# nbip/IWAE

Hardware: AMD Instinct MI355X
Metric: images/sec (train step) IWAE k=50 batch 1024 @1/2/4/8 GPU; test LLH@k=5000 (higher is better)
Workload: dtype bf16; 1 GPU; 1-layer IWAE k=50 batch 1024 per GPU (BASELINE configs[1]; N=8 is configs[4]), objective iwae_elbo, train step = forward + backward + Adam(eps=1e-4); config_id=c1, global_batch=1024, n_samples=50, parallelism=dp1, rccl_ranks=0, settle_steps=100, full=False

## Files before the change

iwae_amd/csrc/kernels.h:

```cpp
#pragma once
#include <hip/hip_runtime.h>
#include <stdint.h>

namespace iwae {

#define IWAE_DENSE_G1_DEFAULT 29u
enum { EPI_TANH = 0, EPI_HEAD = 1, EPI_DX = 2, EPI_F32 = 3, EPI_BERN = 4, EPI_SIGMOID = 5 };
enum { OBJ_VAE_ELBO = 0, OBJ_IWAE_ELBO = 1, OBJ_IWAE_EQ14 = 2, OBJ_VAE_ELBO_KL = 3, OBJ_DREG = 4 };
enum { PB_LME = 0, PB_MEAN, PB_EQ14, PB_KL, PB_PX, PB_T1, PB_T2, PB_DREG, PB_COUNT };
enum { SC_VAE_ELBO = 0, SC_VAE_ELBO_KL, SC_IWAE_ELBO, SC_IWAE_EQ14, SC_INFERENCE_LOSS, SC_MEAN_LPXZ, SC_MEAN_T1, SC_MEAN_T2, SC_KL, SC_COUNT = 16 };

struct EpsSrc {
    const float* user = nullptr;
    const float* cache = nullptr;
    int ldC = 0;
    int B = 0;
    uint64_t seed = 0;
    uint64_t row_offset = 0;
    uint32_t step = 0;
    uint32_t stream = 0;
    int k_total = 0, s_off = 0, kc = 0;
};

struct LseArgs {
// ... 98 lines not shown
};
struct BlockBwdArgs {
    const uint16_t* DH; int ldDH;
    const char *imgH, *imgL2;
    int KTH, KT1, NT1;
    int R;
    const uint16_t *H2, *H1; int ldH;
    uint16_t *D2, *D1;
    int lat_on;
    LatentBwdArgs lat;
    int rows_per_wg;
};
bool block_bwd_ok(const BlockBwdArgs& a);
void launch_block_bwd(const BlockBwdArgs& a, hipStream_t st);
bool block_fwd_ok(const BlockFwdArgs& a);
bool block_fwd_shape_ok(const BlockFwdArgs& a);
void launch_block_fwd(const BlockFwdArgs& a, hipStream_t st);

struct OutBwdArgs {
    const uint16_t* G2; int ldG;
    const char* img1;
    const char* img2;
    int Xdim; int Xp32;
    const float* gx;
    const uint16_t* XB; int ldXB; int k;
    int M, KT, NG;
    uint16_t* DLP;
    const uint16_t* SP;
    float* part; int gpb;
    uint16_t* DPP;
    unsigned long long* stamps;
    int dbg;
};

struct DecBwdArgs {
    OutBwdArgs o;
    const char* imgB2;
    const uint16_t* G1;
    uint16_t* D1P;
    const char* imgB1; int MG1;
    float* DZ; int ldDZ;
    uint16_t* DZH;
    int nw;
};

struct WgradPArgs {
    const uint16_t* X; int ldX; int IT;
    const uint16_t* G; int ldG; int JT;
    int M, rows_per_split;
    float* slabW;
    float* slabB;
    const char* zero;
    const float* rowscale;
    int dbg;
    unsigned long long* stamps;
};

#define WGR_MAX_JOBS 6
struct WgradRowsJob {
    const uint16_t* X; int ldX;
    const uint16_t* G; int ldG;
    int R;
    const float* rowscale;
    int sub0, sub1, split;
    int ib, jb, wg_begin;
};
struct WgradPGroup {
    WgradPArgs a[3];
    int n;
    int gx[3], gy[3];
    int zbeg[4];
};

struct Chain2FwdArgs {
    uint16_t* Z1P;
    float* lqz1x;
    const char *e_img1, *e_img2, *e_imgh;
    const char *d_img1, *d_img2, *d_imgh;
    int M, k, B, D0, D1;
    uint16_t *EH1, *EH2;
    float* EHEAD;
    uint16_t* Z2P;
    uint16_t *DH1, *DH2;
    float* DHEAD;
    const float* head1; int ldH1;
    EpsSrc eps1, eps2;
    float *lpz1z2, *lpz2, *lqz2z1;
};
bool chain2_fwd_ok(int KT0, int KTH, int KT1, int M);
void launch_chain2_fwd(const Chain2FwdArgs& a, hipStream_t st);

struct GBlockBwdArgs {
    const char* imgH;
    const char *imgBh, *imgB2, *imgB1;
    const uint16_t *H2, *H1;
    const float* gx;
    int M, k, B, D;
    EpsSrc eps;
    const float* head1; int ldH1;
    const float* DZIN;
    uint16_t* DHP;
    uint16_t *D2P, *D1P;
    float* DZ2;
    uint16_t* DZD;
    const float* DZDEC;
    int ldDZDEC;
// ... 354 lines not shown
```

iwae_amd/csrc/kernels.hip:

```cpp
#include <hip/hip_runtime.h>
#include <hip/hip_ext.h>
#include <stdint.h>
#include <string.h>
#include <type_traits>
#include <algorithm>
#include "kernels.h"
#include "layout.h"
#include "device_helpers.h"

#ifdef IWAE_DIAG
#define WG_DBG(a, bit) (((a).dbg & (bit)) != 0)
#else
#define WG_DBG(a, bit) false
#endif
namespace iwae {

__device__ __forceinline__ void eps4(const EpsSrc& e, int b, int s, int row, int d4, int D, float n[4]) {
    if (e.cache) {
        const float4 v = *(const float4*)(e.cache + (size_t)row * e.ldC + 4 * d4);
        n[0] = v.x; n[1] = v.y; n[2] = v.z; n[3] = v.w;
    } else if (e.user) {
        const float* p = e.user + ((size_t)s * e.B + b) * D + 4 * d4;
#pragma unroll
        for (int i = 0; i < 4; ++i) n[i] = (4 * d4 + i < D) ? p[i] : 0.0f;
// ... 2905 lines not shown
            }
        }
    }
}

template <int NW, int IGC, int AI, int BJ, bool SC>
__global__ __launch_bounds__(NW * 64, (AI * BJ > 16) ? 2 : NW / 4) void wgradp_kernel(WgradPArgs a) {
    int bx = blockIdx.x, by = blockIdx.y, bz = blockIdx.z;
    const int gx = gridDim.x, gy = gridDim.y, nb = gx * gy * (int)gridDim.z;
    if ((nb & 7) == 0) {
        const int L = bx + gx * (by + gy * bz);
        const int V = (L & 7) * (nb >> 3) + (L >> 3);
        bx = V % gx; by = (V / gx) % gy; bz = V / (gx * gy);
    }
    wgradp_body<NW, IGC, AI, BJ, SC>(a, bx, by, bz);
}

__device__ __forceinline__ void wait_vmem_but_ws(int n) {
#define IWAE_WS_CASE(k) case k: asm volatile("s_waitcnt vmcnt(" #k ")" ::: "memory"); break;
    switch (n) {
        IWAE_WS_CASE(0) IWAE_WS_CASE(1) IWAE_WS_CASE(2) IWAE_WS_CASE(3) IWAE_WS_CASE(4) IWAE_WS_CASE(5) IWAE_WS_CASE(6) IWAE_WS_CASE(7)
        IWAE_WS_CASE(8) IWAE_WS_CASE(9) IWAE_WS_CASE(10) IWAE_WS_CASE(11) IWAE_WS_CASE(12) IWAE_WS_CASE(13) IWAE_WS_CASE(14) IWAE_WS_CASE(15)
        IWAE_WS_CASE(16) IWAE_WS_CASE(17) IWAE_WS_CASE(18) IWAE_WS_CASE(19) IWAE_WS_CASE(20) IWAE_WS_CASE(21) IWAE_WS_CASE(22) IWAE_WS_CASE(23)
        default: asm volatile("s_waitcnt vmcnt(24)" ::: "memory"); break;
    }
#undef IWAE_WS_CASE
}
#ifdef IWAE_DENSE_STAMPS
#define WS_STAMP(slot)                                                                 \
    {                                                                                  \
        unsigned long long t_;                                                         \
        __builtin_amdgcn_sched_barrier(0);                                             \
        asm volatile("s_memtime %0\n\ts_waitcnt lgkmcnt(0)" : "=s"(t_)::"memory");     \
        __builtin_amdgcn_sched_barrier(0);                                             \
        ws_sum[slot] += t_ - ws_prev;                                                  \
        ws_prev = t_;                                                                  \
    }
#define WS_STAMP_OUT()                                                                                                         \
    if (a.stamps && lane == 0) {                                                                                               \
        for (int i_ = 0; i_ < 8; ++i_) a.stamps[((size_t)sid * (NCW + NLW) + wave) * 8 + i_] = ws_sum[i_];                     \
    }
#else
#define WS_STAMP(slot)
#define WS_STAMP_OUT()
#endif
__device__ __forceinline__ void wgradws_block(int& bx, int& bz, const int gx, const int nz) {
    const int nb = gx * nz;
    if ((nb & 7) == 0) {
        const int L = bx + gx * bz;
        const int V = (L & 7) * (nb >> 3) + (L >> 3);
        bx = V % gx; bz = V / gx;
    }
}
template <bool SC, int BJ, int NLW>
__device__ __forceinline__ void wgradws_body(const WgradPArgs& a, const int jt0, const int bz, const int sid) {
    extern __shared__ __attribute__((aligned(1024))) char smem[];
#ifdef IWAE_DENSE_STAMPS
    unsigned long long ws_sum[8] = {0, 0, 0, 0, 0, 0, 0, 0}, ws_prev = 0;
    asm volatile("s_memtime %0\n\ts_waitcnt lgkmcnt(0)" : "=s"(ws_prev)::"memory");
#endif
    constexpr int AI = 7, IGC = 2, NCW = 8, STRIP = 4 * BJ;
    constexpr int XT_BYTES = WG_SR * 512, GROW = STRIP * 32, GT_BYTES = WG_SR * GROW, BUF = XT_BYTES + GT_BYTES;
    constexpr int XP = XT_BYTES / 1024, GP = GT_BYTES / 1024, XPL = XP / NLW, GPL = GP / NLW, PPL = XPL + GPL;
    constexpr int SPR = GROW / 16, RPP = 1024 / GROW;
    static_assert(XP % NLW == 0 && GP % NLW == 0 && GPL >= 1 && GPL <= 4, "loader split");
    typedef __attribute__((ext_vector_type(4))) short v4s;
    auto gswz = [](int r) { return SPR >= 16 ? ((r & 3) << 2) : (((r >> 1) & 1) << 2); };
    const int tid = threadIdx.x, lane = tid & 63, wave = __builtin_amdgcn_readfirstlane(tid >> 6);
    const int rbeg = bz * a.rows_per_split;
    const int rend = min(a.M, rbeg + a.rows_per_split);
    const int nstage = (rend - rbeg + WG_SR - 1) / WG_SR;
    const int gcol0 = jt0 * 16;

    if (SC && wave >= NCW) {
        typedef __attribute__((ext_vector_type(4))) uint32_t u32x4;
        __builtin_amdgcn_s_setprio(3);
        const int lw = wave - NCW;
        const char* zsrc = a.zero + (lane & 31) * 16;
        const int xstride = WG_SR * a.ldX * 2, gstride = WG_DBG(a, 32) ? 0 : WG_SR * a.ldG * 2;
        const char* xbase[XPL]; int xlim[XPL];
#pragma unroll
        for (int i = 0; i < XPL; ++i) {
            const int pc = lw * XPL + i, rl = 2 * pc + (lane >> 5);
            const int col = ((lane & 31) ^ ((rl & 3) << 2)) * 8;
            xbase[i] = (const char*)a.X + ((size_t)(rbeg + rl) * a.ldX + col) * 2;
            xlim[i] = col < a.ldX ? rend - rbeg - rl : -(1 << 30);
        }
        const char* gbase[GPL]; int glim[GPL];
#pragma unroll
        for (int i = 0; i < GPL; ++i) {
            const int pc = lw * GPL + i, rl = RPP * pc + lane / SPR;
            const int col = gcol0 + ((lane % SPR) ^ gswz(rl)) * 8;
            const bool ok = col < a.ldG;
            gbase[i] = (const char*)a.G + ((size_t)(rbeg + rl) * a.ldG + (ok ? col : 0)) * 2;
            glim[i] = ok ? rend - rbeg - rl : -(1 << 30);
        }
        constexpr int NR = RPP * GPL;
        static_assert(NR == 8 || NR == 4, "row weights of a loader and stage are one s_load_dwordx8 / x4");
        typedef __attribute__((ext_vector_type(NR))) float wvec_t;
        auto load_w = [&](int st, wvec_t& w) {
            const uint64_t ad = (uint64_t)(a.rowscale + (rbeg + st * WG_SR + NR * lw));
            const uint64_t au = ((uint64_t)(uint32_t)__builtin_amdgcn_readfirstlane((int)(uint32_t)(ad >> 32)) << 32) |
                                (uint64_t)(uint32_t)__builtin_amdgcn_readfirstlane((int)(uint32_t)ad);
            if constexpr (NR == 8) asm volatile("s_load_dwordx8 %0, %1, 0x0" : "=s"(w) : "s"(au) : "memory");
            else asm volatile("s_load_dwordx4 %0, %1, 0x0" : "=s"(w) : "s"(au) : "memory");
        };
        auto wsel = [&](const wvec_t& w, int i) {
            float f = w[RPP * i];
#pragma unroll
            for (int r = 1; r < RPP; ++r) f = (lane / SPR == r) ? w[RPP * i + r] : f;
            return f;
        };
        constexpr int PER = GPL + XPL;
        u32x4 gq0[GPL], gq1[GPL], gq2[GPL], gq3[GPL];
        auto issue_g = [&](int st, int i, u32x4& dst) {
// ... 22 lines not shown
            for (int i = 0; i < XPL; ++i) issue_x(st, i);
        };
        if (0 < nstage) issue_all(0, gq0);
        if (1 < nstage) issue_all(1, gq1);
        if (2 < nstage) issue_all(2, gq2);
        wait_vmem_but_ws(per_stage(1) + per_stage(2));
        asm volatile("s_waitcnt lgkmcnt(0)" : "+s"(wcur) : : "memory");
        if (0 < nstage) {
#pragma unroll
            for (int i = 0; i < GPL; ++i) { asm volatile("" : "+v"(gq0[i])); put_piece(0, i, gq0[i], wcur); }
        }
        __syncthreads();
        WS_STAMP(0)
        auto iter = [&](int c, u32x4 (&gn)[GPL], u32x4 (&gc)[GPL]) {
            const bool next = c + 1 < nstage;
            if (next) load_w(c + 1, wcur);
            if (c + 3 < nstage) issue_all(c + 3, gn);
            WS_STAMP(1)
            if (next) {
                wait_vmem_but_ws(per_stage(c + 2) + per_stage(c + 3));
                asm volatile("s_waitcnt lgkmcnt(0)" : "+s"(wcur) : : "memory");
            }
            WS_STAMP(2)
            if (next) {
#pragma unroll
                for (int i = 0; i < GPL; ++i) { asm volatile("" : "+v"(gc[i])); put_piece(c + 1, i, gc[i], wcur); }
            }
            WS_STAMP(3)
            __syncthreads();
            WS_STAMP(4)
        };
        for (int c = 0; c < nstage; c += 4) {
            iter(c, gq3, gq1);
            if (c + 1 < nstage) iter(c + 1, gq0, gq2);
            if (c + 2 < nstage) iter(c + 2, gq1, gq3);
            if (c + 3 < nstage) iter(c + 3, gq2, gq0);
        }
        asm volatile("s_waitcnt vmcnt(0)" ::: "memory");
        WS_STAMP_OUT()
        return;
    }
    if (wave >= NCW) {
        const int lw = wave - NCW;
        const char* zsrc = a.zero + (lane & 31) * 16;
        const char* pbase[PPL];
        int plim[PPL];
        const int xstride = WG_SR * a.ldX * 2, gstride = WG_SR * a.ldG * 2;
#pragma unroll
        for (int i = 0; i < PPL; ++i) {
            const bool isx = i < XPL;
            int rl, col, ld;
            if (isx) {
                const int pc = lw * XPL + i;
                rl = 2 * pc + (lane >> 5);
                col = ((lane & 31) ^ ((rl & 3) << 2)) * 8;
                ld = a.ldX;
            } else {
                const int pc = lw * GPL + (i - XPL);
                rl = RPP * pc + lane / SPR;
                col = gcol0 + ((lane % SPR) ^ gswz(rl)) * 8;
                ld = a.ldG;
            }
            pbase[i] = (const char*)(isx ? a.X : a.G) + ((size_t)(rbeg + rl) * ld + col) * 2;
            plim[i] = col < ld ? rend - rbeg - rl : -(1 << 30);
        }
        auto issue = [&](int st) {
#pragma unroll
            for (int i = 0; i < PPL; ++i) {
                const bool isx = i < XPL;
                const int pc = isx ? lw * XPL + i : XP + lw * GPL + (i - XPL);
                const char* src = (st * WG_SR < plim[i]) ? pbase[i] + (size_t)st * (size_t)(isx ? xstride : gstride) : zsrc;
                glds16(src, (uint32_t)__builtin_amdgcn_readfirstlane((int)(lds_addr_of(smem + (st % WG_NST) * BUF) + (uint32_t)pc * 1024u)));
            }
        };
        if (0 < nstage) issue(0);
        if (1 < nstage) issue(1);
        if (2 < nstage) issue(2);
        wait_vmem_but_ws((1 < nstage ? PPL : 0) + (2 < nstage ? PPL : 0));
        __syncthreads();
        for (int c = 0; c < nstage; ++c) {
            const bool refill = c + 3 < nstage && !WG_DBG(a, 1);
            if (refill) issue(c + 3);
            if (c + 1 < nstage) wait_vmem_but_ws((c + 2 < nstage ? PPL : 0) + (refill ? PPL : 0));
            __syncthreads();
        }
        asm volatile("s_waitcnt vmcnt(0)" ::: "memory");
        return;
    }

    const int q = lane >> 4, l16 = lane & 15, qp = l16 >> 2, p = l16 & 3;
    const int ig = wave % IGC, jg = wave / IGC;
    f32x4 acc[AI][BJ], accb[BJ];
#pragma unroll
    for (int u = 0; u < BJ; ++u) {
        accb[u] = (f32x4){0.0f, 0.0f, 0.0f, 0.0f};
#pragma unroll
        for (int t = 0; t < AI; ++t) acc[t][u] = (f32x4){0.0f, 0.0f, 0.0f, 0.0f};
    }
    const int xrow_off = (4 * q + qp) * 512, grow_off = (4 * q + qp) * GROW;
    const uint4 ones = make_uint4(0x3F803F80u, 0x3F803F80u, 0x3F803F80u, 0x3F803F80u);
    const bool do_bias = ig == 0 && !WG_DBG(a, 4);
    __syncthreads();
    WS_STAMP(0)
    for (int c = 0; c < nstage; ++c) {
        const int buf = c % WG_NST;
        const char* xb = smem + buf * BUF + xrow_off + p * 16;
        const char* gbase = smem + buf * BUF + XT_BYTES + grow_off;
        uint4 g[BJ];
#pragma unroll
        for (int u = 0; u < BJ; ++u) {
            const int jl = jg * BJ + u;
            const char* gb = gbase + ((((4 * (jl >> 1)) ^ gswz(qp)) + p) * 16) + 8 * (jl & 1);
            const v4s g0 = __builtin_amdgcn_ds_read_tr16_b64_v4i16((__attribute__((address_space(3))) v4s*)gb);
            const v4s g1 = __builtin_amdgcn_ds_read_tr16_b64_v4i16((__attribute__((address_space(3))) v4s*)(gb + 16 * GROW));
            const uint2 glo = __builtin_bit_cast(uint2, g0), ghi = __builtin_bit_cast(uint2, g1);
            g[u] = make_uint4(glo.x, glo.y, ghi.x, ghi.y);
        }
        WS_STAMP(1)
        if (!WG_DBG(a, 2)) {
            lds_pipeline<AI, 3>(
                [&](int t) {
                    const int i = ig * AI + t;
                    const char* p0 = xb + ((((4 * (i >> 1)) ^ (qp << 2))) * 16) + 8 * (i & 1);
                    const v4s r0 = __builtin_amdgcn_ds_read_tr16_b64_v4i16((__attribute__((address_space(3))) v4s*)p0);
                    const v4s r1 = __builtin_amdgcn_ds_read_tr16_b64_v4i16((__attribute__((address_space(3))) v4s*)(p0 + 16 * 512));
                    const uint2 lo = __builtin_bit_cast(uint2, r0), hi = __builtin_bit_cast(uint2, r1);
                    return make_uint4(lo.x, lo.y, hi.x, hi.y);
                },
                [&](int t, const uint4& av) {
#pragma unroll
                    for (int u = 0; u < BJ; ++u) acc[t][u] = mfma16(av, g[u], acc[t][u]);
                });
        }
        if (do_bias) {
#pragma unroll
            for (int u = 0; u < BJ; ++u) accb[u] = mfma16(ones, g[u], accb[u]);
        }
        WS_STAMP(2)
        __syncthreads();
        WS_STAMP(3)
    }
    if (WG_DBG(a, 16)) return;
    float* slab = a.slabW + (size_t)bz * a.IT * 16 * a.JT * 16;
#pragma unroll
    for (int u = 0; u < BJ; ++u) {
        const int jt = jt0 + jg * BJ + u;
        if (jt < a.JT) {
#pragma unroll
            for (int t = 0; t < AI; ++t) {
                const int it = ig * AI + t;
                if (it < a.IT) {
#pragma unroll
                    for (int ii = 0; ii < 4; ++ii)
                        slab[(size_t)(it * 16 + 4 * q + ii) * (a.JT * 16) + jt * 16 + l16] = acc[t][u][ii];
                }
            }
            if (ig == 0 && q == 0) a.slabB[(size_t)bz * a.JT * 16 + jt * 16 + l16] = accb[u][0];
        }
    }
    WS_STAMP(4)
    WS_STAMP_OUT()
}

template <bool SC, int BJ, int NLW>
__global__ __launch_bounds__((8 + NLW) * 64, NLW == 8 ? 4 : 3) void wgradws_kernel(WgradPArgs a) {
    int bx = blockIdx.x, bz = blockIdx.z;
    wgradws_block(bx, bz, gridDim.x, gridDim.z);
    const int sid = bz * (int)gridDim.x + bx;
    if constexpr (BJ == 4) {
        if (bx == (int)gridDim.x - 1 && a.JT - bx * 16 <= 4 && (SC || gridDim.x > 1)) { wgradws_body<SC, 1, NLW>(a, bx * 16, bz, sid); return; }
    }
    wgradws_body<SC, BJ, NLW>(a, bx * 4 * BJ, bz, sid);
}
__global__ __launch_bounds__(768, 3) void wgradws_group_kernel(WgradPGroup g) {
    int l = 0;
    while (l + 1 < g.n && (int)blockIdx.z >= g.zbeg[l + 1]) ++l;
    if ((int)blockIdx.x >= g.gx[l]) return;
    int bx = blockIdx.x, bz = blockIdx.z - g.zbeg[l];
    wgradws_block(bx, bz, g.gx[l], g.zbeg[l + 1] - g.zbeg[l]);
    wgradws_body<false, 4, 4>(g.a[l], bx * 16, bz, 0);
}

__global__ __launch_bounds__(512, 2) void wgradp_group_kernel(WgradPGroup g) {
    int l = 0;
    while (l + 1 < g.n && (int)blockIdx.z >= g.zbeg[l + 1]) ++l;
    if ((int)blockIdx.x >= g.gx[l] || (int)blockIdx.y >= g.gy[l]) return;
    wgradp_body<8, 4, 4, 4, false>(g.a[l], blockIdx.x, blockIdx.y, blockIdx.z - g.zbeg[l]);
}
__global__ __launch_bounds__(512, 2) void wgradp_group_sc_kernel(WgradPGroup g) {
    int l = 0;
    while (l + 1 < g.n && (int)blockIdx.z >= g.zbeg[l + 1]) ++l;
    if ((int)blockIdx.x >= g.gx[l] || (int)blockIdx.y >= g.gy[l]) return;
    if (l == 0) wgradp_body<8, 4, 4, 4, true>(g.a[0], blockIdx.x, blockIdx.y, blockIdx.z);
    else wgradp_body<8, 4, 4, 4, false>(g.a[l], blockIdx.x, blockIdx.y, blockIdx.z - g.zbeg[l]);
}

__global__ __launch_bounds__(256) void prep_rows_kernel(const float* x, const float* cond, int B, int X, int C, int Xp, int Bp, uint16_t* XP) {
    const int lane = threadIdx.x & 63;
    const int b = blockIdx.x * 64 + lane;
    const int nchunk = Xp / 8;
    if (b >= Bp) return;
    for (int c = blockIdx.y * 4 + (threadIdx.x >> 6); c < nchunk; c += gridDim.y * 4) {
        const int t = c >> 2, qq = c & 3;
        float v[8];
#pragma unroll
        for (int h = 0; h < 2; ++h) {
            const int f0 = 32 * t + 16 * h + 4 * qq;
#pragma unroll
            for (int i = 0; i < 4; ++i) {
                const int f = f0 + i;
                float t = 0.0f;
                if (b < B && f < X) t = x[(size_t)b * X + f];
                else if (b < B && f < X + C) t = cond[(size_t)b * C + (f - X)];
                v[4 * h + i] = t;
            }
        }
        if (b < B) *(uint4*)(XP + (size_t)b * Xp + 8 * c) = make_uint4(pack2(v[0], v[1]), pack2(v[2], v[3]), pack2(v[4], v[5]), pack2(v[6], v[7]));
    }
}

__global__ __launch_bounds__(256) void gather_binarize_kernel(const uint8_t* data, const int32_t* order, int start, int N, int B, int X, int Xp,
                                                              int Bp, uint64_t seed, uint32_t epoch, uint16_t* XP, float* xf,
                                                              const uint8_t* labels, int C, float* cond_out) {
    const int lane = threadIdx.x & 63;
    const int b = blockIdx.x * 64 + lane;
    const int nchunk = Xp / 8;
    if (b >= Bp) return;
    const int img = (b < B) ? order[start + b] : 0;
    const int lab = (labels && b < B) ? (int)labels[img] : -1;
    if (cond_out && blockIdx.y == 0 && threadIdx.x < 64 && b < B)
        for (int j = 0; j < C; ++j) cond_out[(size_t)b * C + j] = (j == lab) ? 1.0f : 0.0f;
    for (int c = blockIdx.y * 4 + (threadIdx.x >> 6); c < nchunk; c += gridDim.y * 4) {
        const int t = c >> 2, qq = c & 3;
// ... 858 lines not shown
        const int nparts = a.part ? (a.NG + a.gpb - 1) / a.gpb : 1;
        dim3 grid((a.M + 127) / 128, nparts);
        hipEvent_t stop = g_stop_event;
        if (a.part) g_stop_event = nullptr;
        switch (a.KT) {
            case 7: LAUNCH_EV(out_bwd_s_kernel<7>, grid, dim3(256), lds, st, a); break;
            case 4: LAUNCH_EV(out_bwd_s_kernel<4>, grid, dim3(256), lds, st, a); break;
            case 2: LAUNCH_EV(out_bwd_s_kernel<2>, grid, dim3(256), lds, st, a); break;
            default: return;
        }
        if (a.part) {
            g_stop_event = stop;
            LAUNCH_EV(out_bwd_finish_kernel, grid1((size_t)a.M * (a.ldG / 8), 256), dim3(256), 0, st, a, nparts);
        }
        return;
    }
    constexpr int PAIRS = 2;
    const size_t ldsp = 2 * ((size_t)a.KT * 4096 + 1024) + (size_t)PAIRS * 4096;
    dim3 gridp((a.M + PAIRS * 32 - 1) / (PAIRS * 32));
#ifdef IWAE_DIAG
    if (a.stamps) {
        LAUNCH_EV((out_bwd_pair_kernel<7, PAIRS, true>), gridp, dim3(PAIRS * 128), 2 * ((size_t)7 * 4096 + 1024) + (size_t)PAIRS * 4096, st, a);
        return;
    }
#endif
    switch (a.KT) {
        case 7: LAUNCH_EV((out_bwd_pair_kernel<7, PAIRS, false>), gridp, dim3(PAIRS * 128), ldsp, st, a); break;
        case 4: LAUNCH_EV((out_bwd_pair_kernel<4, PAIRS, false>), gridp, dim3(PAIRS * 128), ldsp, st, a); break;
        case 2: LAUNCH_EV((out_bwd_pair_kernel<2, PAIRS, false>), gridp, dim3(PAIRS * 128), ldsp, st, a); break;
        default: {
            const size_t lds = 2 * ((size_t)a.KT * 8192 + 1024);
            LAUNCH_EV((out_bwd_kernel<0, false>), dim3((a.M + 127) / 128), dim3(256), lds, st, a);
        }
    }
}
void launch_wgradws_group(const WgradPGroup& g, hipStream_t st) {
    int mx = 0;
    for (int l = 0; l < g.n; ++l) mx = std::max(mx, g.gx[l]);
    LAUNCH_EV(wgradws_group_kernel, dim3(mx, 1, g.zbeg[g.n]), dim3(768), WG_NST * (WG_SR * 512 + WG_SR * 512), st, g);
}
void launch_wgradp_group(const WgradPGroup& g, hipStream_t st) {
    int mx = 0, my = 0;
    for (int l = 0; l < g.n; ++l) { mx = std::max(mx, g.gx[l]); my = std::max(my, g.gy[l]); }
    if (g.a[0].rowscale) hipLaunchKernelGGL(wgradp_group_sc_kernel, dim3(mx, my, g.zbeg[g.n]), dim3(512), WG_NST * (WG_SR * 512 + WG_SR * 256 + 1024), st, g);
    else hipLaunchKernelGGL(wgradp_group_kernel, dim3(mx, my, g.zbeg[g.n]), dim3(512), WG_NST * (WG_SR * 512 + WG_SR * 256), st, g);
}
int wgradp_strip(int shape) { return (shape == 8 || shape == 9) ? 8 : 16; }
void launch_wgradp(const WgradPArgs& a, int nsplit, int shape, hipStream_t st) {
    dim3 grid((a.JT + wgradp_strip(shape) - 1) / wgradp_strip(shape), (a.IT + 15) / 16, nsplit);
    const size_t sc = a.rowscale ? 1024 : 0;
    if (shape == 7) {
        const size_t lds = WG_NST * (WG_SR * 512 + WG_SR * 512);
        if (a.rowscale) LAUNCH_EV((wgradws_kernel<true, 4, 4>), grid, dim3(768), lds, st, a);
        else LAUNCH_EV((wgradws_kernel<false, 4, 4>), grid, dim3(768), lds, st, a);
    } else if (shape == 9) {
        const size_t lds = WG_NST * (WG_SR * 512 + WG_SR * 256);
        if (a.rowscale) LAUNCH_EV((wgradws_kernel<true, 2, 8>), grid, dim3(1024), lds, st, a);
        else LAUNCH_EV((wgradws_kernel<false, 2, 8>), grid, dim3(1024), lds, st, a);
    } else if (shape == 16) {
        const size_t lds = WG_NST * (WG_SR * 512 + WG_SR * 512 + sc);
        if (a.rowscale) LAUNCH_EV((wgradp_kernel<16, 2, 8, 2, true>), grid, dim3(1024), lds, st, a);
        else LAUNCH_EV((wgradp_kernel<16, 4, 4, 4, false>), grid, dim3(1024), lds, st, a);
    } else {
        const size_t lds = WG_NST * (WG_SR * 512 + WG_SR * 256 + sc);
        if (a.rowscale) LAUNCH_EV((wgradp_kernel<8, 4, 4, 4, true>), grid, dim3(512), lds, st, a);
        else LAUNCH_EV((wgradp_kernel<8, 4, 4, 4, false>), grid, dim3(512), lds, st, a);
    }
}
void launch_prep_rows(const float* x, const float* cond, int B, int X, int C, int Xp, int Bp, uint16_t* XP, hipStream_t st) {
    const int nchunk = Xp / 8;
    hipLaunchKernelGGL(prep_rows_kernel, dim3(Bp / 64, std::min(32, (nchunk + 3) / 4)), dim3(256), 0, st, x, cond, B, X, cond ? C : 0, Xp, Bp, XP);
}
void launch_gather_binarize(const uint8_t* data, const int32_t* order, int start, int N, int B, int X, int Xp, int Bp, uint64_t seed,
                            uint32_t epoch, uint16_t* XP, float* xf, hipStream_t st, const uint8_t* labels, int C, float* cond_out) {
    const int nchunk = Xp / 8;
    hipLaunchKernelGGL(gather_binarize_kernel, dim3(Bp / 64, std::min(32, (nchunk + 3) / 4)), dim3(256), 0, st, data, order, start, N, B, X, Xp,
                       Bp, seed, epoch, XP, xf, labels, labels ? C : 0, cond_out);
}
void launch_eps_gen_multi(const EpsSrc& e, int M, int D, int ld, float* out, int nsteps, size_t step_stride, hipStream_t st) {
    const int nd4 = (D + 3) / 4;
    hipLaunchKernelGGL(eps_gen_multi_kernel, grid1((size_t)nsteps * M * nd4, 256), dim3(256), 0, st, e, M, nd4, ld, out, nsteps, step_stride);
}
void launch_eps_gen(const EpsSrc& e, int M, int D, int ld, float* out, hipStream_t st, int max_blocks) {
    const int nd4 = (D + 3) / 4;
    dim3 grid = grid1((size_t)M * nd4, 256);
    if (max_blocks > 0 && (int)grid.x > max_blocks) grid.x = max_blocks;
    hipLaunchKernelGGL(eps_gen_kernel, grid, dim3(256), 0, st, e, M, nd4, ld, out);
}
void launch_sample(const SampleArgs& a, hipStream_t st) { hipLaunchKernelGGL(sample_kernel, dim3((a.M + 63) / 64), dim3(256), 0, st, a); }
void launch_gauss_lp(const GaussLpArgs& a, hipStream_t st) { hipLaunchKernelGGL(gauss_lp_kernel, dim3((a.M + 63) / 64), dim3(256), 0, st, a); }
void launch_lse(const LseArgs& a, hipStream_t st) {
    if (a.k >= 2048) LAUNCH_EV(lse_block_kernel<16>, dim3(a.B), dim3(1024), 0, st, a);
    else if (a.k > 256) LAUNCH_EV(lse_block_kernel<4>, dim3(a.B), dim3(256), 0, st, a);
    else LAUNCH_EV(lse_kernel, grid1((size_t)a.B * 64, 256), dim3(256), 0, st, a);
}
void launch_latent_bwd(const LatentBwdArgs& a, hipStream_t st) {
    if (a.dzh && !a.dz2 && a.eps.cache && !a.prior_head) hipLaunchKernelGGL(latent_bwd_kernel<1>, dim3(a.Bp), dim3(256), 0, st, a);
    else if (!a.dzh && a.dz && a.dz2 && a.dz3 && a.eps.cache && !a.prior_head) hipLaunchKernelGGL(latent_bwd_kernel<2>, dim3(a.Bp), dim3(256), 0, st, a);
    else hipLaunchKernelGGL(latent_bwd_kernel<0>, dim3(a.Bp), dim3(256), 0, st, a);
}
void launch_gauss_bwd(const GaussBwdArgs& a, hipStream_t st) {
    hipLaunchKernelGGL(gauss_bwd_kernel, grid1((size_t)a.Mp * (a.Dp / 4), 256), dim3(256), 0, st, a);
}
void launch_reduce_grads(const LayerDesc* layers, int nlayers, int first_block, int nblocks, float* grad, float* param, float* mom, float* vel,
                         float alpha, float beta1, float beta2, float eps, int fuse_adam, const float* per_b, int B, float beta, float* scalars, hipStream_t st,
                         int first_block2, int nblocks2) {
// ... 50 lines not shown
```

iwae_amd/csrc/model.h:

```cpp
#pragma once
#include <hip/hip_runtime.h>
#include <stddef.h>
#include <stdint.h>
#include <string>
#include <type_traits>
#include <vector>
#include <rccl/rccl.h>
#include "../../include/iwae_amd.h"
#include "kernels.h"

#pragma GCC visibility push(hidden)

int fail(int code, const std::string& msg);
#define HIPCHK(expr)                                                                                   \
    do {                                                                                               \
        hipError_t e_ = (expr);                                                                        \
        if (e_ != hipSuccess)                                                                          \
            return fail(e_ == hipErrorOutOfMemory ? IWAE_ERR_NOMEM : IWAE_ERR_HIP,                     \
                        std::string(#expr) + ": " + hipGetErrorString(e_));                            \
    } while (0)
#define CHK(expr) do { int rc_ = (expr); if (rc_ != IWAE_OK) return rc_; } while (0)

struct DevBuf { void* p = nullptr; size_t cap = 0; };
struct KerasLayer { std::string name; int Kin, Nout; size_t offW, offb; };
// ... 23 lines not shown

enum TimedKernel { T_OUT_BWD = 0, T_DEC_FWD, T_WGRAD_OUT, T_DX_HID, T_DX_LAT, T_WGRAD_HID, T_WGRAD_LAT, T_LATENT_BWD, T_ENC_FWD, T_REDUCE, T_DEC_BWD, T_AR_ENC, T_AR_DEC, T_AIS_CHAIN, T_LOCAL_Q, T_IMPUTE, T_COUNT };

struct FwdCall {
    uint32_t batch_offset = 0;
    int cond_row0 = 0;
    int k_total = 0, s_off = 0;
    bool log_w_only = false;
    bool no_ksplit = false;
};

struct StepOptions {
    bool allow_s_mode = true;
    bool allow_zin = true;
    bool allow_zin_eval = false;
    bool allow_eps_multi = true;
    int eps_blocks = 512;
    bool allow_block_fused = true;
    bool allow_out_in_block = true;
    bool allow_dec_fused = true;
    bool allow_bern_pipe = true;
    bool bern_qw = true;
    bool bern_qw_force = false;
    bool allow_lse_fused = true;
    bool allow_lse_dup = true;
    bool allow_lse_in_bwd = true;
    bool allow_early_wout = true;
    bool allow_g2w = false;
    bool allow_chain2 = true;
    bool allow_chain2_bwd = true;
    unsigned dense_g1_mask = IWAE_DENSE_G1_DEFAULT;
    bool allow_dec_bwd = true;
    bool small_dec_bwd = true; int small_rows = 8191;
    int dec_rows_max = 1024;
    int dec_bwd_nw = 8;
    bool allow_dz_half = true;
    bool allow_wg3 = true;
    bool allow_dec_rows = true;
    bool allow_wgrad_rows = true;
    bool allow_lat_rows4 = false;
    bool allow_lat_in_block = true;
    bool use_side2 = true;
    bool allow_wg_group = false;
    int wout_split = 0, wout_wg1 = 56, wout_wg2 = 128;
    bool defer_split = false;
    bool allow_defer = true;
    bool allow_defer2 = true;
    bool allow_defer2_split = true;
    int wg_target16 = 0;
    int wg_target16_1 = 64;
    int wg_target8 = 128;
    int wg_target8_few = 32;
    int wg_shape9 = 0;
    bool allow_wg7 = true;
    bool dp_concurrent = false;
    iwae::GemmF32Opts gemm_f32;
    bool allow_f32_multi_reduce = true;
    bool allow_f32_side = true, f32_wout_first = true;
    int f32_dw_last = 0;
    int f32_dw_min_rows = 32;
    int f32_dw_tiles = 1024;
    bool f32_dec_fused_train = false;
    bool allow_f32_dec_fused = true;
    bool allow_f32_bern_fused = true;
    int eval_rows = 0;
    int grid_chunk = 0;
    int ais_t_chunk = 0;
    int local_t_chunk = 0;
    int impute_rows = 0;
};

enum ZFrom { Z_SAMPLE = 0, Z_DENSE_ZIN, Z_DEC_PROLOGUE, Z_BLOCK, Z_CHAIN2 };
enum DecFwd { DEC_DENSE = 0, DEC_BLOCK2, DEC_BLOCK_OUT, DEC_PIPE };
enum LseAt { LSE_FWD = 0, LSE_DECODER, LSE_BWD_ROWS };
enum DxPath { DX_THREE = 0, DX_DEC_BWD, DX_ROWS };
enum OnStream { ON_MAIN = 0, ON_SIDE, ON_SIDE2 };
struct StepPlan {
    bool zin_eval = false;
    bool keep_eps = false;
    bool eps_multi = false;
    bool enc_takes_f32 = false;
    ZFrom z_from = Z_SAMPLE;
    bool chain = false;
    bool chain2_bwd = false;
    DecFwd dec_fwd = DEC_DENSE;
    iwae::DenseArgs bern;
    iwae::BlockFwdArgs dec_blk;
    int px_parts = 1;
    bool s_mode = false;
    bool early_wout = false;
    bool lse_fused = false;
    bool lse_dup = false;
    bool g2w = false;
    LseAt lse_at = LSE_FWD;
    bool want_dreg = false;
    OnStream draw_on = ON_SIDE;
    bool dec_rows = false;
    DxPath dx = DX_THREE;
    iwae::DecBwdRowsArgs rows;
    bool out_parts = false;
    bool dz_half = false;
    bool lat_fuse = false;
    bool rows_enc = false;
    bool group3 = false;
    bool wout_two_part = false;
    bool hid_group = false;
// ... 213 lines not shown
```

iwae_amd/csrc/model.hip:

```cpp
#include <math.h>
#include <stdio.h>
#include <string.h>
#include <stddef.h>
#include <stdlib.h>
#include <algorithm>
#include <random>
#include <memory>
#include <dlfcn.h>
#include "model.h"
#include "layout.h"

using namespace iwae;

static_assert(sizeof(iwae_config) == 64 && offsetof(iwae_config, struct_size) == 0 && offsetof(iwae_config, seed) == 32 && offsetof(iwae_config, cond_dim) == 48 &&
              offsetof(iwae_config, cond_prior) == 52 && offsetof(iwae_config, precision) == 56, "iwae_config layout is part of the ABI (iwae_amd/_capi.py)");
static_assert(sizeof(iwae_scalars) == 64 && sizeof(iwae_tensors) == 12 * sizeof(void*), "ABI struct layout");
static_assert(sizeof(iwae_ais_options) == 72 && offsetof(iwae_ais_options, betas) == 16 && offsetof(iwae_ais_options, step_size) == 24 && offsetof(iwae_ais_options, z0) == 40 &&
              offsetof(iwae_ais_options, unif) == 64 && sizeof(iwae_ais_outputs) == 10 * sizeof(void*), "iwae_ais_options / iwae_ais_outputs layout is part of the ABI (iwae_amd/_capi.py)");
static_assert(sizeof(iwae_local_options) == 64 && offsetof(iwae_local_options, objective) == 16 && offsetof(iwae_local_options, lr) == 20 && offsetof(iwae_local_options, epsilon) == 32 &&
              offsetof(iwae_local_options, mu0) == 40 && offsetof(iwae_local_options, eps) == 56 && sizeof(iwae_local_outputs) == 9 * sizeof(void*), "iwae_local_options / iwae_local_outputs layout is part of the ABI (iwae_amd/_capi.py)");
static_assert(sizeof(iwae_impute_options) == 24 && offsetof(iwae_impute_options, k) == 4 && offsetof(iwae_impute_options, mask) == 8 && offsetof(iwae_impute_options, eps) == 16 &&
              sizeof(iwae_impute_outputs) == 6 * sizeof(void*), "iwae_impute_options / iwae_impute_outputs layout is part of the ABI (iwae_amd/_capi.py)");

static thread_local std::string g_err;
// ... 224 lines not shown
    e.cache = m->epsc_ptr[layer];
    e.ldC = eps_ld(m, layer);
    if (m->user_eps) e.user = ptr<float>(m->epsbuf) + (layer == 0 ? 0 : (size_t)m->k * m->B * m->D[0]);
    e.B = m->B;
    e.seed = m->cfg.seed;
    e.row_offset = (uint64_t)m->call.batch_offset * (uint64_t)m->k;
    e.step = m->noise_step;
    e.stream = (uint32_t)layer;
    if (m->call.k_total > 0) {
        e.k_total = m->call.k_total; e.s_off = m->call.s_off; e.kc = m->k;
        e.row_offset = (uint64_t)m->call.batch_offset * (uint64_t)m->call.k_total;
    }
    return e;
}
namespace {

int attach_dense_stamps(iwae_model* m, int epi, DenseArgs& a) {
    if (m->dstamp_epi != epi || m->dstamp_kt != a.KT || (a.M < 4096 && a.KT <= 8)) return IWAE_OK;
    m->dstamp_waves = std::max(((a.M + 127) / 128) * ((a.MG + a.mg_per_block - 1) / a.mg_per_block) * 4, epi == EPI_BERN ? ((a.M + 127) / 128) * 16 : 0);
    CHK(ensure(m->dstamps, (size_t)m->dstamp_waves * 64, m->stream));
    a.stamps = ptr<unsigned long long>(m->dstamps);
    return IWAE_OK;
}

bool block_fwd_shape(const iwae_model* m, const Linear* blk, int R, BlockFwdArgs& a) {
    memset(&a, 0, sizeof(a));
    a.ldX = blk[0].Kp32; a.img0 = blk[0].imgF; a.img1 = blk[1].imgF; a.img2 = blk[2].imgF;
    a.KT0 = blk[0].KT; a.KT1 = blk[1].KT; a.NT1 = blk[0].Np32 / 16; a.NT2 = blk[2].Np32 / 16; a.R = R;
    a.ldH = blk[0].Np32; a.ldYF = blk[2].Np32; a.split = (blk[2].nsub == 2) ? blk[2].joff[1] : (1 << 30);
    return m->opt.allow_block_fused && blk[1].Np32 == blk[0].Np32 && blk[2].KT == blk[1].KT && blk[1].Kp32 == blk[0].Np32 && block_fwd_ok(a);
}

void wgradp_shape(const iwae_model* m, const Linear& L, int rows, int& nsplit, int& nw, int& cps) {
    const int chunks = (rows + 63) / 64;
    nw = (L.JT > 8 && chunks >= 128) ? 16 : 8;
    if (nw == 16 && L.IT <= 14 && m->opt.allow_wg7) nw = (m->opt.wg_shape9 & (L.JT > 16 ? 1 : 2)) ? 9 : 7;
    const int blocks = ((L.JT + wgradp_strip(nw) - 1) / wgradp_strip(nw)) * ((L.IT + 15) / 16);
    const int target16 = m->opt.wg_target16 > 0 ? m->opt.wg_target16 : (m->cfg.n_layers == 2 ? 64 : 96);
    const int target = (nw != 8) ? (blocks == 1 ? m->opt.wg_target16_1 : target16) : (chunks < 128 ? m->opt.wg_target8_few : m->opt.wg_target8);
    nsplit = std::max(1, std::min(chunks, target / std::max(1, blocks)));
    cps = (chunks + nsplit - 1) / nsplit;
    nsplit = (chunks + cps - 1) / cps;
}
int wgradp_plan(iwae_model* m, Linear& L, const uint16_t* XP, const uint16_t* GP, int rows, WgradPArgs& a, int& nsplit, int& nw) {
    int cps;
    wgradp_shape(m, L, rows, nsplit, nw, cps);
    const size_t needW = (size_t)nsplit * L.IT * 16 * L.JT * 16 * 4, needB = (size_t)nsplit * L.JT * 16 * 4;
    void* oldW = L.slabW.p; void* oldB = L.slabB.p;
    CHK(ensure(L.slabW, needW, m->stream));
    CHK(ensure(L.slabB, needB, m->stream));
    if (oldW != L.slabW.p || oldB != L.slabB.p || nsplit != L.nsplit) { L.nsplit = nsplit; m->descs_dirty = true; }
    a.X = XP; a.ldX = L.Kp32; a.IT = L.IT; a.G = GP; a.ldG = L.Np32; a.JT = L.JT; a.M = rows; a.rows_per_split = cps * 64;
    a.slabW = ptr<float>(L.slabW); a.slabB = ptr<float>(L.slabB); a.zero = m->d_zero; a.rowscale = nullptr;
    a.dbg = m->wg_debug;
    a.stamps = nullptr;
    return IWAE_OK;
}

int wgradp(iwae_model* m, Linear& L, const uint16_t* XP, const uint16_t* GP, int rows, hipStream_t st = nullptr,
           const float* rowscale = nullptr) {
    WgradPArgs a;
    int nsplit = 1, nw = 8;
    CHK(wgradp_plan(m, L, XP, GP, rows, a, nsplit, nw));
    a.rowscale = rowscale;
    if (rowscale && (m->fake_s & 2)) a.dbg |= 32;
#ifdef IWAE_DENSE_STAMPS
    if (m->dstamp_epi == 10 && rowscale && nw == 7) {
        m->dstamp_waves = ((L.JT + 15) / 16) * nsplit * 12;
        CHK(ensure(m->dstamps, (size_t)m->dstamp_waves * 64, m->stream));
        a.stamps = ptr<unsigned long long>(m->dstamps);
    }
#endif
    launch_wgradp(a, nsplit, nw, st ? st : m->stream);
    HIPCHK(hipGetLastError());
    return IWAE_OK;
}

int wgradp_two_plan(iwae_model* m, Linear& L, const uint16_t* XP, const uint16_t* GP, int rows, const float* rowscale, WgradPArgs& a1, int& n1, WgradPArgs& a2, int& n2) {
    const int blocks = (L.JT + 15) / 16;
    const int chunks = (rows + 63) / 64;
    const int c1 = std::min(chunks - 1, std::max(1, (int)((long)chunks * m->opt.wout_split / 100)));
    const int c2 = chunks - c1;
    auto split = [&](int ch, int target, int& n, int& cps) { n = std::max(1, std::min(ch, target / std::max(1, blocks))); cps = (ch + n - 1) / n; n = (ch + cps - 1) / cps; };
    int cps1, cps2;
    split(c1, m->opt.wout_wg1, n1, cps1);
    split(c2, m->opt.wout_wg2, n2, cps2);
    const int ns = n1 + n2;
    const size_t stride = (size_t)L.IT * 16 * L.JT * 16;
    void* oldW = L.slabW.p; void* oldB = L.slabB.p;
    CHK(ensure(L.slabW, (size_t)ns * stride * 4, m->stream));
    CHK(ensure(L.slabB, (size_t)ns * L.JT * 16 * 4, m->stream));
    if (oldW != L.slabW.p || oldB != L.slabB.p || ns != L.nsplit) { L.nsplit = ns; m->descs_dirty = true; }
    const int R1 = c1 * 64;
    memset(&a1, 0, sizeof(a1));
    a1.X = XP; a1.ldX = L.Kp32; a1.IT = L.IT; a1.G = GP; a1.ldG = L.Np32; a1.JT = L.JT; a1.M = R1; a1.rows_per_split = cps1 * 64;
    a1.slabW = ptr<float>(L.slabW); a1.slabB = ptr<float>(L.slabB); a1.zero = m->d_zero; a1.rowscale = rowscale;
    a2 = a1;
    a2.X = XP + (size_t)R1 * L.Kp32; a2.G = GP + (size_t)R1 * L.Np32; a2.M = rows - R1; a2.rows_per_split = cps2 * 64;
    a2.slabW = a1.slabW + (size_t)n1 * stride; a2.slabB = a1.slabB + (size_t)n1 * L.JT * 16; a2.rowscale = rowscale + R1;
    return IWAE_OK;
}

int dense_dx(iwae_model* m, Linear& L, const uint16_t* GP, int rows, const uint16_t* ACT, uint16_t* YP, float* YF) {
    DenseArgs a;
    memset(&a, 0, sizeof(a));
    a.X = GP; a.ldX = L.Np32; a.img = L.imgB;
// ... 1361 lines not shown
    HIPCHK(hipSetDevice(m->cfg.device));
    CHK(join_side(m));
    HIPCHK(hipStreamSynchronize(m->stream));
    if (m->side) HIPCHK(hipStreamSynchronize(m->side));
    if (m->side2) HIPCHK(hipStreamSynchronize(m->side2));
    m->have_forward = false;
    const bool on = value != 0;
    const int iv = (int)value;
    const std::string n(name);
    if (n == "out_recompute") m->opt.allow_s_mode = !on;
    else if (n == "no_defer") m->opt.allow_defer = !on;
    else if (n == "wout_split") m->opt.wout_split = std::max(0, std::min(95, iv));
    else if (n == "wout_wg1") m->opt.wout_wg1 = std::max(1, iv);
    else if (n == "wout_wg2") m->opt.wout_wg2 = std::max(1, iv);
    else if (n == "defer_split") m->opt.defer_split = on;
    else if (n == "no_eps_multi") m->opt.allow_eps_multi = !on;
    else if (n == "no_zin") m->opt.allow_zin = !on;
    else if (n == "zin_eval") m->opt.allow_zin_eval = on;
    else if (n == "no_chain2_bwd") m->opt.allow_chain2_bwd = !on;
    else if (n == "no_chain2") m->opt.allow_chain2 = !on;
    else if (n == "no_dec_bwd") m->opt.allow_dec_bwd = !on;
    else if (n == "no_defer2_split") m->opt.allow_defer2_split = !on;
    else if (n == "no_defer2") m->opt.allow_defer2 = !on;
    else if (n == "f32_dw_tiles") m->opt.f32_dw_tiles = std::max(1, iv);
    else if (n == "f32_dw_min_rows") m->opt.f32_dw_min_rows = std::max(16, iv);
    else if (n == "f32_gemm_dbg") m->opt.gemm_f32.dbg = iv;
    else if (n == "f32_gemm_small_min") m->opt.gemm_f32.v2_small_min = std::max(1, iv);
    else if (n == "f32_ksplit_min_tiles") m->opt.gemm_f32.ksplit_min_tiles = std::max(1, iv);
    else if (n == "f32_no_ksplit") m->opt.gemm_f32.ksplit = !on;
    else if (n == "f32_gemm_small_v1") m->opt.gemm_f32.v2_small = !on;
    else if (n == "f32_gemm_w4") m->opt.gemm_f32.w8 = !on;
    else if (n == "f32_gemm_v1") m->opt.gemm_f32.v2 = !on;
    else if (n == "no_f32_side") m->opt.allow_f32_side = !on;
    else if (n == "f32_dw_last") m->opt.f32_dw_last = iv;
    else if (n == "f32_wout_last") m->opt.f32_wout_first = !on;
    else if (n == "no_f32_multi_reduce") m->opt.allow_f32_multi_reduce = !on;
    else if (n == "f32_dec_fused_train") m->opt.f32_dec_fused_train = on;
    else if (n == "no_f32_dec_fused") m->opt.allow_f32_dec_fused = !on;
    else if (n == "no_f32_bern_fused") m->opt.allow_f32_bern_fused = !on;
    else if (n == "no_dec_rows") m->opt.allow_dec_rows = !on;
    else if (n == "no_wgrad_rows") m->opt.allow_wgrad_rows = !on;
    else if (n == "no_wg3") m->opt.allow_wg3 = !on;
    else if (n == "g2w") m->opt.allow_g2w = on;
    else if (n == "lat_rows4") m->opt.allow_lat_rows4 = on;
    else if (n == "no_lat_in_block") m->opt.allow_lat_in_block = !on;
    else if (n == "no_lse_in_bwd") m->opt.allow_lse_in_bwd = !on;
    else if (n == "no_lse_fused") m->opt.allow_lse_fused = !on;
    else if (n == "no_lse_dup") m->opt.allow_lse_dup = !on;
    else if (n == "dz_f32") m->opt.allow_dz_half = !on;
    else if (n == "no_small_dec_bwd") m->opt.small_dec_bwd = !on;
    else if (n == "small_rows") m->opt.small_rows = iv;
    else if (n == "dec_rows") m->opt.dec_rows_max = iv;
    else if (n == "no_wg7") m->opt.allow_wg7 = !on;
    else if (n == "wg9") m->opt.wg_shape9 = iv;
    else if (n == "grid_chunk") m->opt.grid_chunk = iv > 0 ? std::max(16, iv) : 0;
    else if (n == "ais_t_chunk") m->opt.ais_t_chunk = iv > 0 ? iv : 0;
    else if (n == "local_t_chunk") m->opt.local_t_chunk = iv > 0 ? iv : 0;
    else if (n == "impute_rows") m->opt.impute_rows = iv > 0 ? iv : 0;
    else if (n == "eval_rows") m->opt.eval_rows = iv > 0 ? std::max(64, iv) : 0;
    else if (n == "no_bern_pipe") m->opt.allow_bern_pipe = !on;
    else if (n == "no_block_fused") m->opt.allow_block_fused = !on;
    else if (n == "no_out_in_block") m->opt.allow_out_in_block = !on;
    else if (n == "no_dec_fused") m->opt.allow_dec_fused = !on;
    else if (n == "no_bern_qw") m->opt.bern_qw = !on;
    else if (n == "bern_qw_force") m->opt.bern_qw_force = on;
    else if (n == "dense_g1") m->opt.dense_g1_mask = (unsigned)iv;
    else if (n == "wg8") m->opt.wg_target8 = std::max(1, iv);
    else if (n == "wg8_few") m->opt.wg_target8_few = std::max(1, iv);
    else if (n == "wg16") m->opt.wg_target16 = std::max(1, iv);
    else if (n == "wg16_1") m->opt.wg_target16_1 = std::max(1, iv);
    else if (n == "eps_blocks") m->opt.eps_blocks = std::max(0, iv);
    else if (n == "dec_bwd_nw") m->opt.dec_bwd_nw = iv == 8 ? 8 : 4;
    else if (n == "no_side2") m->opt.use_side2 = !on;
    else if (n == "wg_group") m->opt.allow_wg_group = on;
    else if (n == "no_early_wout") m->opt.allow_early_wout = !on;
    else if (n == "dp_concurrent") m->opt.dp_concurrent = on;
#ifdef IWAE_DIAG
    else if (n == "stamps") { m->want_stamps = on; if (on) { m->opt.allow_s_mode = false; m->opt.allow_bern_pipe = false; m->opt.allow_block_fused = false; m->opt.allow_dec_fused = false; } }
    else if (n == "dense_stamps_epi") m->dstamp_epi = iv;
    else if (n == "dense_stamps_kt") m->dstamp_kt = iv;
    else if (n == "wg_debug") m->wg_debug = iv;
    else if (n == "abl_skip") m->abl_skip = iv;
    else if (n == "fake_s") m->fake_s = iv;
#endif
    else return fail(IWAE_ERR_ARG, "set_option: unknown option '" + n + "'");
    return IWAE_OK;
}

int iwae_set_eval_precision(iwae_handle m, int32_t precision) {
    if (!m) return fail(IWAE_ERR_ARG, "null handle");
    if (precision != IWAE_PREC_BF16 && precision != IWAE_PREC_FP32) return fail(IWAE_ERR_ARG, "precision must be IWAE_PREC_BF16 or IWAE_PREC_FP32");
    m->eval_precision = precision;
    return IWAE_OK;
}

int iwae_set_adam(iwae_handle m, float beta1, float beta2, float epsilon) {
    if (!m) return fail(IWAE_ERR_ARG, "null handle");
    if (!(beta1 >= 0.f && beta1 < 1.f) || !(beta2 >= 0.f && beta2 < 1.f) || !(epsilon > 0.f)) return fail(IWAE_ERR_ARG, "set_adam: need 0 <= beta < 1, epsilon > 0");
    m->adam_b1 = beta1; m->adam_b2 = beta2; m->adam_eps = epsilon;
    return IWAE_OK;
}

int iwae_train_step(iwae_handle m, const float* x, int32_t B, int32_t k, float beta, float lr, int32_t objective, const float* eps,
                    iwae_scalars* scalars, const iwae_tensors* want) {
    if (!m) return fail(IWAE_ERR_ARG, "null handle");
    HIPCHK(hipSetDevice(m->cfg.device));
// ... 487 lines not shown
```

Baseline: 5.193 million images/s.

## Add narrow-X tile variant to weight-gradient kernel for small input widths

New measurement: 5.265 million images/s (median of 6 runs). 1.01x the previous value.

```diff
diff --git a/iwae_amd/csrc/kernels.h b/iwae_amd/csrc/kernels.h
--- a/iwae_amd/csrc/kernels.h
+++ b/iwae_amd/csrc/kernels.h
@@ -174,6 +174,7 @@
     float* slabB;
     const char* zero;
     const float* rowscale;
+    int narrow_x;
     int dbg;
     unsigned long long* stamps;
 };
diff --git a/iwae_amd/csrc/kernels.hip b/iwae_amd/csrc/kernels.hip
--- a/iwae_amd/csrc/kernels.hip
+++ b/iwae_amd/csrc/kernels.hip
@@ -2981,15 +2981,18 @@
         bx = V % gx; bz = V / gx;
     }
 }
-template <bool SC, int BJ, int NLW>
+template <bool SC, int BJ, int NLW, bool NX = false>
 __device__ __forceinline__ void wgradws_body(const WgradPArgs& a, const int jt0, const int bz, const int sid) {
     extern __shared__ __attribute__((aligned(1024))) char smem[];
 #ifdef IWAE_DENSE_STAMPS
     unsigned long long ws_sum[8] = {0, 0, 0, 0, 0, 0, 0, 0}, ws_prev = 0;
     asm volatile("s_memtime %0\n\ts_waitcnt lgkmcnt(0)" : "=s"(ws_prev)::"memory");
 #endif
-    constexpr int AI = 7, IGC = 2, NCW = 8, STRIP = 4 * BJ;
-    constexpr int XT_BYTES = WG_SR * 512, GROW = STRIP * 32, GT_BYTES = WG_SR * GROW, BUF = XT_BYTES + GT_BYTES;
+    constexpr int AI = NX ? 8 : 7, IGC = NX ? 1 : 2, NCW = 8, STRIP = 4 * BJ;
+    constexpr int BJW = STRIP / (NCW / IGC);
+    constexpr int XPITCH = NX ? 256 : 512, XSL = XPITCH / 16, XRPP = 1024 / XPITCH;
+    static_assert(!NX || (!SC && BJ == 4), "the narrow X tile exists for the unweighted 8 + 4-wave shape");
+    constexpr int XT_BYTES = WG_SR * XPITCH, GROW = STRIP * 32, GT_BYTES = WG_SR * GROW, BUF = XT_BYTES + GT_BYTES;
     constexpr int XP = XT_BYTES / 1024, GP = GT_BYTES / 1024, XPL = XP / NLW, GPL = GP / NLW, PPL = XPL + GPL;
     constexpr int SPR = GROW / 16, RPP = 1024 / GROW;
     static_assert(XP % NLW == 0 && GP % NLW == 0 && GPL >= 1 && GPL <= 4, "loader split");
@@ -3118,8 +3121,8 @@
             int rl, col, ld;
             if (isx) {
                 const int pc = lw * XPL + i;
-                rl = 2 * pc + (lane >> 5);
-                col = ((lane & 31) ^ ((rl & 3) << 2)) * 8;
+                rl = XRPP * pc + lane / XSL;
+                col = ((lane % XSL) ^ ((rl & 3) << 2)) * 8;
                 ld = a.ldX;
             } else {
                 const int pc = lw * GPL + (i - XPL);
@@ -3156,14 +3159,14 @@
 
     const int q = lane >> 4, l16 = lane & 15, qp = l16 >> 2, p = l16 & 3;
     const int ig = wave % IGC, jg = wave / IGC;
-    f32x4 acc[AI][BJ], accb[BJ];
-#pragma unroll
-    for (int u = 0; u < BJ; ++u) {
+    f32x4 acc[AI][BJW], accb[BJW];
+#pragma unroll
+    for (int u = 0; u < BJW; ++u) {
         accb[u] = (f32x4){0.0f, 0.0f, 0.0f, 0.0f};
 #pragma unroll
         for (int t = 0; t < AI; ++t) acc[t][u] = (f32x4){0.0f, 0.0f, 0.0f, 0.0f};
     }
-    const int xrow_off = (4 * q + qp) * 512, grow_off = (4 * q + qp) * GROW;
+    const int xrow_off = (4 * q + qp) * XPITCH, grow_off = (4 * q + qp) * GROW;
     const uint4 ones = make_uint4(0x3F803F80u, 0x3F803F80u, 0x3F803F80u, 0x3F803F80u);
     const bool do_bias = ig == 0 && !WG_DBG(a, 4);
     __syncthreads();
@@ -3172,10 +3175,10 @@
         const int buf = c % WG_NST;
         const char* xb = smem + buf * BUF + xrow_off + p * 16;
         const char* gbase = smem + buf * BUF + XT_BYTES + grow_off;
-        uint4 g[BJ];
-#pragma unroll
-        for (int u = 0; u < BJ; ++u) {
-            const int jl = jg * BJ + u;
+        uint4 g[BJW];
+#pragma unroll
+        for (int u = 0; u < BJW; ++u) {
+            const int jl = jg * BJW + u;
             const char* gb = gbase + ((((4 * (jl >> 1)) ^ gswz(qp)) + p) * 16) + 8 * (jl & 1);
             const v4s g0 = __builtin_amdgcn_ds_read_tr16_b64_v4i16((__attribute__((address_space(3))) v4s*)gb);
             const v4s g1 = __builtin_amdgcn_ds_read_tr16_b64_v4i16((__attribute__((address_space(3))) v4s*)(gb + 16 * GROW));
@@ -3189,18 +3192,18 @@
                     const int i = ig * AI + t;
                     const char* p0 = xb + ((((4 * (i >> 1)) ^ (qp << 2))) * 16) + 8 * (i & 1);
                     const v4s r0 = __builtin_amdgcn_ds_read_tr16_b64_v4i16((__attribute__((address_space(3))) v4s*)p0);
-                    const v4s r1 = __builtin_amdgcn_ds_read_tr16_b64_v4i16((__attribute__((address_space(3))) v4s*)(p0 + 16 * 512));
+                    const v4s r1 = __builtin_amdgcn_ds_read_tr16_b64_v4i16((__attribute__((address_space(3))) v4s*)(p0 + 16 * XPITCH));
                     const uint2 lo = __builtin_bit_cast(uint2, r0), hi = __builtin_bit_cast(uint2, r1);
                     return make_uint4(lo.x, lo.y, hi.x, hi.y);
                 },
                 [&](int t, const uint4& av) {
 #pragma unroll
-                    for (int u = 0; u < BJ; ++u) acc[t][u] = mfma16(av, g[u], acc[t][u]);
+                    for (int u = 0; u < BJW; ++u) acc[t][u] = mfma16(av, g[u], acc[t][u]);
                 });
         }
         if (do_bias) {
 #pragma unroll
-            for (int u = 0; u < BJ; ++u) accb[u] = mfma16(ones, g[u], accb[u]);
+            for (int u = 0; u < BJW; ++u) accb[u] = mfma16(ones, g[u], accb[u]);
         }
         WS_STAMP(2)
         __syncthreads();
@@ -3209,8 +3212,8 @@
     if (WG_DBG(a, 16)) return;
     float* slab = a.slabW + (size_t)bz * a.IT * 16 * a.JT * 16;
 #pragma unroll
-    for (int u = 0; u < BJ; ++u) {
-        const int jt = jt0 + jg * BJ + u;
+    for (int u = 0; u < BJW; ++u) {
+        const int jt = jt0 + jg * BJW + u;
         if (jt < a.JT) {
 #pragma unroll
             for (int t = 0; t < AI; ++t) {
@@ -3228,7 +3231,7 @@
     WS_STAMP_OUT()
 }
 
-template <bool SC, int BJ, int NLW>
+template <bool SC, int BJ, int NLW, bool NX = false>
 __global__ __launch_bounds__((8 + NLW) * 64, NLW == 8 ? 4 : 3) void wgradws_kernel(WgradPArgs a) {
     int bx = blockIdx.x, bz = blockIdx.z;
     wgradws_block(bx, bz, gridDim.x, gridDim.z);
@@ -3236,7 +3239,7 @@
     if constexpr (BJ == 4) {
         if (bx == (int)gridDim.x - 1 && a.JT - bx * 16 <= 4 && (SC || gridDim.x > 1)) { wgradws_body<SC, 1, NLW>(a, bx * 16, bz, sid); return; }
     }
-    wgradws_body<SC, BJ, NLW>(a, bx * 4 * BJ, bz, sid);
+    wgradws_body<SC, BJ, NLW, NX>(a, bx * 4 * BJ, bz, sid);
 }
 __global__ __launch_bounds__(768, 3) void wgradws_group_kernel(WgradPGroup g) {
     int l = 0;
@@ -3244,7 +3247,8 @@
     if ((int)blockIdx.x >= g.gx[l]) return;
     int bx = blockIdx.x, bz = blockIdx.z - g.zbeg[l];
     wgradws_block(bx, bz, g.gx[l], g.zbeg[l + 1] - g.zbeg[l]);
-    wgradws_body<false, 4, 4>(g.a[l], bx * 16, bz, 0);
+    if (g.a[l].narrow_x) wgradws_body<false, 4, 4, true>(g.a[l], bx * 16, bz, 0);
+    else wgradws_body<false, 4, 4>(g.a[l], bx * 16, bz, 0);
 }
 
 __global__ __launch_bounds__(512, 2) void wgradp_group_kernel(WgradPGroup g) {
@@ -4209,6 +4213,7 @@
     if (shape == 7) {
         const size_t lds = WG_NST * (WG_SR * 512 + WG_SR * 512);
         if (a.rowscale) LAUNCH_EV((wgradws_kernel<true, 4, 4>), grid, dim3(768), lds, st, a);
+        else if (a.narrow_x) LAUNCH_EV((wgradws_kernel<false, 4, 4, true>), grid, dim3(768), lds, st, a);
         else LAUNCH_EV((wgradws_kernel<false, 4, 4>), grid, dim3(768), lds, st, a);
     } else if (shape == 9) {
         const size_t lds = WG_NST * (WG_SR * 512 + WG_SR * 256);
diff --git a/iwae_amd/csrc/model.h b/iwae_amd/csrc/model.h
--- a/iwae_amd/csrc/model.h
+++ b/iwae_amd/csrc/model.h
@@ -99,6 +99,7 @@
     int wg_target8 = 128;
     int wg_target8_few = 32;
     int wg_shape9 = 0;
+    bool wg_narrow_x = true;
     bool allow_wg7 = true;
     bool dp_concurrent = false;
     iwae::GemmF32Opts gemm_f32;
diff --git a/iwae_amd/csrc/model.hip b/iwae_amd/csrc/model.hip
--- a/iwae_amd/csrc/model.hip
+++ b/iwae_amd/csrc/model.hip
@@ -300,6 +300,7 @@
     if (oldW != L.slabW.p || oldB != L.slabB.p || nsplit != L.nsplit) { L.nsplit = nsplit; m->descs_dirty = true; }
     a.X = XP; a.ldX = L.Kp32; a.IT = L.IT; a.G = GP; a.ldG = L.Np32; a.JT = L.JT; a.M = rows; a.rows_per_split = cps * 64;
     a.slabW = ptr<float>(L.slabW); a.slabB = ptr<float>(L.slabB); a.zero = m->d_zero; a.rowscale = nullptr;
+    a.narrow_x = m->opt.wg_narrow_x && L.Kp32 <= 128 && L.IT <= 8;
     a.dbg = m->wg_debug;
     a.stamps = nullptr;
     return IWAE_OK;
@@ -1767,6 +1768,7 @@
     else if (n == "small_rows") m->opt.small_rows = iv;
     else if (n == "dec_rows") m->opt.dec_rows_max = iv;
     else if (n == "no_wg7") m->opt.allow_wg7 = !on;
+    else if (n == "wg_narrow_x") m->opt.wg_narrow_x = on;
     else if (n == "wg9") m->opt.wg_shape9 = iv;
     else if (n == "grid_chunk") m->opt.grid_chunk = iv > 0 ? std::max(16, iv) : 0;
     else if (n == "ais_t_chunk") m->opt.ais_t_chunk = iv > 0 ? iv : 0;
```
